# ChangwuLiu/InGVIO

Hardware: AMD Instinct MI355X
Metric: ekf_updates_per_sec (higher is better)
Workload: dtype f64; 1 GPU; BASELINE configs[1]: synthetic stereo MSCKF, 150 feats x 11 clones, state dim N=249 (update at N), 512 independent filters per GPU; step = propagate(k=10)+clone+MSCKF update+marginalise; filters_per_gpu=512, feats=150, clones=11, state_dim=249, imu_steps=10, parallelism=independent filters, 1 rank(s), no data-path collective

## Files before the change

include/ingvio_hip.h:

```cpp
#ifndef INGVIO_HIP_H
#define INGVIO_HIP_H

#include <stddef.h>

#ifdef __cplusplus
extern "C" {
#endif

#define INGVIO_OK 0
#define INGVIO_NO_ROWS 1
#define INGVIO_NEG_DIAG 2
#define INGVIO_REJECTED 3
#define INGVIO_E_ARG (-1)
#define INGVIO_E_CAPACITY (-2)
#define INGVIO_E_HIP (-3)
#define INGVIO_E_NOT_IN_STATE (-4)
#define INGVIO_E_UNSUPPORTED (-5)
#define INGVIO_E_NOT_PD (-6)

typedef struct ingvio_ctx ingvio_ctx;

typedef struct {
    int batch;
    int n_max;
// ... 302 lines not shown
    int track;
    int anchor;
    double pf[3];
} ingvio_lm_init_cand;
typedef struct {
    int n_cand; const ingvio_lm_init_cand* cand;
    int n_drop; const int* drop_cols;
} ingvio_lm_init_block;
int ingvio_landmark_init_nominal(ingvio_ctx* ctx, int b0, int nb, const ingvio_lm_init_block* blocks, const ingvio_msckf_opts* opts,
                                 double chi2_mult, int do_chi2, int cand_cap,
                                 int* added, int* new_idx, int* slot, double* chi2, double* dx, int* status);
int ingvio_debug_landmark_init_rows(ingvio_ctx* ctx, int b, const ingvio_lm_init_cand* cand, const ingvio_msckf_opts* opts,
                                    int n_drop, const int* drop_cols, double* H_old, double* H_new, double* res, int* m_out);
int ingvio_frame_run(ingvio_ctx* ctx, int restore_prior);
int ingvio_set_frame_parts(ingvio_ctx* ctx, int parts);
int ingvio_frame_fetch(ingvio_ctx* ctx, int b0, int nb, double* dx_out, int* accepted, int* rows_out);
int ingvio_frame_fetch_begin(ingvio_ctx* ctx, int b0, int nb);
int ingvio_frame_fetch_end(ingvio_ctx* ctx, double* dx_out, int* accepted, int* rows_out);

int ingvio_debug_msckf_info(ingvio_ctx* ctx, int b, double* A_out, int* ncol_out);

int ingvio_debug_info_solution(ingvio_ctx* ctx, int b, double* out, int count);

int ingvio_debug_tracks_read(ingvio_ctx* ctx, int b, unsigned long long* mask, double* uv, double* pf);

int ingvio_debug_staged_frame(ingvio_ctx* ctx, int b, int* n_clones, int* n_feat, int* clone_idx, double* clone_R, double* clone_p,
                              int* anchor, int* dof, unsigned long long* obs_mask, double* pf, double* uv);

int ingvio_debug_read(ingvio_ctx* ctx, long long* out, int n);

int ingvio_profile_enable(ingvio_ctx* ctx, int enable);
int ingvio_profile_select(ingvio_ctx* ctx, const char* kernel_name);
int ingvio_profile_reset(ingvio_ctx* ctx);
int ingvio_profile_get(ingvio_ctx* ctx, const char** names, double* ms, int* calls, int cap);

#ifdef __cplusplus
}
#endif
#endif
```

ingvio_amd/capi.py:

```python
import ctypes as C
import os

import numpy as np

_HERE = os.path.dirname(os.path.abspath(__file__))
LIB_PATH = os.environ.get("INGVIO_HIP_LIB") or os.path.join(_HERE, "lib", "libingvio_hip.so")

c_dp = C.POINTER(C.c_double)
c_ip = C.POINTER(C.c_int)
c_up = C.POINTER(C.c_ulonglong)

OK, NO_ROWS, NEG_DIAG, REJECTED = 0, 1, 2, 3
E_ARG, E_CAPACITY, E_HIP, E_NOT_IN_STATE, E_UNSUPPORTED, E_NOT_PD = -1, -2, -3, -4, -5, -6
R_SCALAR, R_DIAG, R_FULL = 0, 1, 2

EXPORTS = [
    "ingvio_ctx_create", "ingvio_ctx_destroy", "ingvio_sync", "ingvio_ctx_stream", "ingvio_f_max", "ingvio_c_max", "ingvio_last_error", "ingvio_ldp",
    "ingvio_build_id",
    "ingvio_cov_set", "ingvio_cov_get", "ingvio_get_n", "ingvio_cov_get_marginal", "ingvio_cov_snapshot",
    "ingvio_cov_restore", "ingvio_propagate", "ingvio_propagate_fused", "ingvio_augment_clone", "ingvio_marginalize",
    "ingvio_append_independent", "ingvio_ekf_update", "ingvio_chi2_gamma", "ingvio_msckf_update", "ingvio_msckf_update_tri", "ingvio_qr_compress",
    "ingvio_frame_stage", "ingvio_frame_stage_async", "ingvio_frame_set_imu_noise", "ingvio_frame_fetch_begin", "ingvio_frame_fetch_end", "ingvio_tracks_create", "ingvio_frame_stage_tracks", "ingvio_frame_run", "ingvio_set_frame_parts", "ingvio_frame_fetch", "ingvio_profile_enable", "ingvio_profile_select",
    "ingvio_profile_reset",
    "ingvio_profile_get", "ingvio_set_msckf_method", "ingvio_set_qr_method", "ingvio_landmark_stage", "ingvio_landmark_run",
    "ingvio_landmark_fetch", "ingvio_frame_run_phase", "ingvio_info_set", "ingvio_debug_read", "ingvio_triangulate",
    "ingvio_gnss_front_stage", "ingvio_gnss_front_fetch", "ingvio_gnss_update_batch", "ingvio_gnss_stage", "ingvio_gnss_run", "ingvio_gnss_fetch", "ingvio_mld", "ingvio_debug_msckf_info", "ingvio_debug_info_solution",
    "ingvio_info_reduce", "ingvio_info_commit", "ingvio_gnss_sat_eval",
    "ingvio_chi2_gamma_multi", "ingvio_ekf_update_batch", "ingvio_add_variable_delayed_invertible", "ingvio_add_variable_delayed", "ingvio_add_variable_delayed_batch", "ingvio_replace_var_linear",
    "ingvio_nominal_create", "ingvio_nominal_set", "ingvio_nominal_get", "ingvio_nominal_box_plus", "ingvio_frame_stage_tracks_nominal",
    "ingvio_nominal_set_gnss", "ingvio_nominal_get_gnss", "ingvio_gnss_front_stage_nominal", "ingvio_landmark_stage_nominal",
    "ingvio_landmark_init_nominal", "ingvio_debug_landmark_init_rows", "ingvio_nominal_tail",
    "ingvio_debug_tracks_read", "ingvio_debug_staged_frame",
]

NOM_NONE, NOM_SE23, NOM_SE3, NOM_VEC3, NOM_SCALAR, NOM_LANDMARK = -1, 0, 1, 2, 3, 4
NOM_VAL = 15

# ... 921 lines not shown
        fn = self.L.ingvio_frame_stage_async if use_async else self.L.ingvio_frame_stage

        def call(_keep=(keeps, chi2, sa, fa, o, sg)):
            self._chk(fn(self.h, b0, nb, sa, fa, C.byref(o), _d(sg), int(enable_gnss), C.c_double(sigma_cb), C.c_double(sigma_rw)))
        return call

    def frame_set_imu_noise(self, b0, noise):
        nz = f64(np.asarray(noise, dtype=np.float64).reshape(-1, 6))
        self._chk(self.L.ingvio_frame_set_imu_noise(self.h, int(b0), nz.shape[0], _d(nz)))

    def frame_run(self, restore_prior=False):
        self._chk(self.L.ingvio_frame_run(self.h, 1 if restore_prior else 0))

    def set_frame_parts(self, parts):
        self._chk(self.L.ingvio_set_frame_parts(self.h, int(parts)))

    def frame_fetch(self, b0=0, nb=None):
        nb = self.batch if nb is None else nb
        dx = np.zeros((nb, self.ldp)); acc = np.zeros((nb, self.f_max), dtype=np.int32); rows = np.zeros(nb, dtype=np.int32)
        self._chk(self.L.ingvio_frame_fetch(self.h, b0, nb, _d(dx), _i(acc), _i(rows)))
        return dx, acc, rows

    def frame_fetch_begin(self, b0=0, nb=None):
        nb = self.batch if nb is None else nb
        self._fetch_nb = nb
        self._chk(self.L.ingvio_frame_fetch_begin(self.h, b0, nb))

    def frame_fetch_end(self):
        nb = self._fetch_nb
        dx = np.empty((nb, self.ldp)); acc = np.empty((nb, self.f_max), dtype=np.int32); rows = np.empty(nb, dtype=np.int32)
# ... 85 lines not shown
```

ingvio_amd/csrc/capi.hip:

```cpp
#include "../../include/ingvio_hip.h"
#include "dev_common.h"
#include "launch_ekf.h"
#include "launch_msckf.h"
#include "launch_factored.h"
#include "launch_tri.h"
#include "launch_tracks.h"
#include "launch_lm.h"
#include "launch_delayed.h"
#include "launch_qr.h"
#include "launch_chol.h"
#include "launch_gnss.h"
#include "launch_lmbatch.h"
#include "launch_nominal.h"
#include "launch_tail.h"

#include <stdio.h>
#include <stdlib.h>
#include <string.h>
#include <unistd.h>
#include <string>
#include <atomic>
#include <cmath>
#include <condition_variable>
#include <functional>
// ... 123 lines not shown
    hipStream_t st2 = nullptr;
    hipEvent_t ev_fork = nullptr, ev_join = nullptr, ev_ref = nullptr;
    hipEvent_t ev_fetch = nullptr;
    int fetch_b0 = 0, fetch_nb = 0;
    hipStream_t st_copy = nullptr;
    hipEvent_t ev_copy = nullptr, ev_free[2] = { nullptr, nullptr };
    bool copy_pending = false, free_valid[2] = { false, false };
    int set_id = 0;
    struct PinSlab { char* p = nullptr; size_t cap = 0; hipEvent_t ev = nullptr; bool busy = false; };
    PinSlab pin[4];
    int pin_next = 0;
    struct PartStream { hipStream_t st = nullptr; hipEvent_t ev_gate = nullptr, ev_apply = nullptr, ev_done = nullptr; };
    PartStream part[4];
    int parts_alloc = 0;
    int parts_req = -1;
    bool split_pending = false;
    hipEvent_t tok_last = nullptr;
    hipEvent_t ev_split_fork = nullptr;
    hipStream_t run_st = nullptr;
    hipEvent_t tok_wait = nullptr, tok_rec = nullptr;
    struct Tracks { double *uv = nullptr, *pf = nullptr; unsigned long long* mask = nullptr; int t_max = 0; char* stage[2] = { nullptr, nullptr }; size_t stage_cap = 0; } trk;
    struct Nominal {
        int vmax = 0, ir = 0, dr = 0;
        int* ih = nullptr; double* dv = nullptr;
        int* ih_snap = nullptr; double* dv_snap = nullptr;
        double* dx = nullptr;
        std::vector<int> h_ih, h_ih_snap;
        bool has_snap = false;
        bool pending = false;
        bool frame = false;
// ... 547 lines not shown
    { ProfScope p(c, PF_EKF_CORE); launch_ekf_core(E, c->run_st); }
    L.gY = E.Y; L.gYstride = ws; L.gm = g.mf + b0;
    g.fused_last = true;
    g.results = true;
    return 0;
}

int run_msckf_factored(ingvio_ctx* c, int b0, int nb, const MsckfOpts& op, int stereo, int fmax_used,
                       const int* marg_idx = nullptr, int marg_size = 0, int phase = 0, bool gnss_fuse = false)
{
    FactoredLaunch L;
    memset(&L, 0, sizeof L);
    L.stereo = stereo; L.cv = view(c); L.fv = fview(c); L.op = op; L.b0 = b0; L.nb = nb;
    L.fmax_used = fmax_used > 0 ? fmax_used : 1;
    L.ncol_cap = 6 * c->d.c_max;
    for (int i = 0; i < nb; ++i) if (c->h_nclones[b0 + i] > L.c_used) L.c_used = c->h_nclones[b0 + i];
    L.gamma = c->d_gamma; L.accept = c->d_accept; L.used = c->d_used; L.rec = c->d_rec;
    L.Apart = c->d_Rpart + (size_t)b0 * c->G * c->rstride; L.chunk_used = c->d_chunk_used + (size_t)b0 * c->G;
    L.G = c->G; L.rstride = c->rstride; L.noise = c->d_noise + b0;
    L.Tflat = c->d_Tflat; L.tfstride = (size_t)c->ldp * 100; L.flat_nb = std::min(c->d.batch, APPLY_FLAT_NB);
    L.Asum = c->d_Asum ? c->d_Asum + (size_t)b0 * c->rstride : nullptr; L.used_sum = c->d_used_sum ? c->d_used_sum + b0 : nullptr;
#ifdef INGVIO_ALT_KERNELS
    static const bool few_off = [] { const char* e = getenv("INGVIO_FEW"); return e && !strcmp(e, "off"); }();
    if (few_off) { L.Tflat = nullptr; L.Asum = nullptr; }
#endif
    L.T = c->d_Y + (size_t)b0 * c->ystride; L.Pc = c->d_Yc + (size_t)b0 * c->ystride; L.ystride = c->ystride;
    L.dx = c->d_dx; L.m_out = c->d_m + b0; L.nc_out = c->d_nc + b0; L.status = c->d_status;
    L.big_sg = c->d_big_sg ? c->d_big_sg + (size_t)b0 * bigwin_sg_doubles(c->G) : nullptr;
    L.big_wk = c->d_big_wk ? c->d_big_wk + (size_t)b0 * bigwin_wk_doubles() : nullptr;
    const bool big = c->d.c_max > 16;
// ... 98 lines not shown
    if (desc->c_max > bigwin_cmax()) return INGVIO_E_CAPACITY;
    if (desc->m_max > 128) return INGVIO_E_CAPACITY;
    int ndev = 0;
    if (hipGetDeviceCount(&ndev) != hipSuccess || ndev <= desc->device) return INGVIO_E_HIP;
    ingvio_ctx* c = new ingvio_ctx();
    c->d = *desc;
    if (c->d.m_max < 1) c->d.m_max = 32;
    c->err.clear();
    if (hipSetDevice(desc->device) != hipSuccess) { delete c; return INGVIO_E_HIP; }
    c->own_stream = desc->stream == nullptr;
    if (c->own_stream) {
        if (hipStreamCreateWithFlags(&c->st, hipStreamNonBlocking) != hipSuccess) { delete c; return INGVIO_E_HIP; }
    } else c->st = (hipStream_t)desc->stream;
    c->run_st = c->st;
    if (const char* e = getenv("INGVIO_FRAME_PARTS")) c->parts_req = atoi(e);
    if (desc->c_max > 16) {
        int lo = 0, hi = 0;
        hipDeviceGetStreamPriorityRange(&lo, &hi);
        if (hipStreamCreateWithPriority(&c->st2, hipStreamNonBlocking, hi) != hipSuccess) c->st2 = nullptr;
        if (c->st2 && (hipEventCreateWithFlags(&c->ev_fork, hipEventDisableTiming) != hipSuccess ||
                       hipEventCreateWithFlags(&c->ev_ref, hipEventDisableTiming) != hipSuccess ||
                       hipEventCreateWithFlags(&c->ev_join, hipEventDisableTiming) != hipSuccess)) { hipStreamDestroy(c->st2); c->st2 = nullptr; }
    }
    const int B = desc->batch;
    c->ldp = (desc->n_max + 15) & ~15;
    const int cls0 = desc->c_max > 16 ? bigwin_cmax() : msckf_cmax_class(desc->c_max);
    const int cpad = cls0 > desc->c_max ? cls0 : desc->c_max;
    const int mcap = c->d.m_max > 6 * cpad ? c->d.m_max : 6 * cpad;
    c->mld = (mcap + 15) & ~15;
    c->nc_cap = c->ldp > mcap ? c->ldp : mcap;
// ... 2956 lines not shown
    if (c->alt_ready) {
        HIPCHK(c, hipEventRecord(c->ev_free[c->set_id], c->st));
        c->free_valid[c->set_id] = true;
    }
    return INGVIO_OK;
}

int ingvio_frame_run(ingvio_ctx* c, int restore_prior) { return frame_run_impl(c, restore_prior, 0); }
int ingvio_set_frame_parts(ingvio_ctx* c, int parts)
{
    if (!c || parts < -1 || parts > 4) return INGVIO_E_ARG;
    ENTER(c);
    c->parts_req = parts == 0 ? 1 : parts;
    return INGVIO_OK;
}
int ingvio_frame_run_phase(ingvio_ctx* c, int restore_prior, int phase)
{
    if (phase < 0 || phase > 2) return INGVIO_E_ARG;
    return frame_run_impl(c, restore_prior, phase);
}

int ingvio_info_set(ingvio_ctx* c, int b, const double* A, int ncol, int n_accepted)
{
    ENTER(c);
    if (check_range(c, b, 1) || !A || ncol < 6 || (size_t)ncol * (ncol + 1) > (size_t)c->rstride || n_accepted < 0) return INGVIO_E_ARG;
    std::vector<int> used(c->G, 0);
    used[0] = n_accepted;
    int rc = up(c, c->d_Rpart + (size_t)b * c->G * c->rstride, A, 8 * (size_t)ncol * (ncol + 1));
    rc |= up(c, c->d_chunk_used + (size_t)b * c->G, used.data(), sizeof(int) * (size_t)c->G);
    if (rc) return INGVIO_E_HIP;
// ... 191 lines not shown
    if (dbg_read_factored(a, 64) || dbg_read_cov(bq, 64) || dbg_read_bigwin(cq, 64) || dbg_read_solve(sq, 64)) return INGVIO_E_HIP;
    long long hq[64];
    if (dbg_read_chol(hq, 64)) return INGVIO_E_HIP;
    long long lq[64], mq[64];
    if (dbg_read_lmbatch(lq, 64) || dbg_read_lmchol(mq, 64)) return INGVIO_E_HIP;
    if (const char* e = getenv("INGVIO_DBG_TU")) {
        const long long* src = e[0] == 'b' ? cq : (e[0] == 'c' ? hq : (e[0] == 's' ? sq : (e[0] == 'l' ? lq : (e[0] == 'm' ? mq : a))));
        for (int i = 0; i < n; ++i) out[i] = src[i];
        return INGVIO_OK;
    }
    for (int i = 0; i < n; ++i)
        out[i] = i >= 56 ? hq[i - 56] : (i >= 48 ? cq[i] : ((i >= 24 && i < 32) ? sq[i - 24] : ((i < 16 || i >= 32) ? a[i] : bq[i])));
    return INGVIO_OK;
}

int ingvio_profile_select(ingvio_ctx* c, const char* kernel_name)
{
    ENTER(c);
    if (!c) return INGVIO_E_ARG;
    c->prof_only = -1;
    if (!kernel_name || !*kernel_name) return INGVIO_OK;
    for (int i = 0; i < PF_COUNT; ++i) if (!strcmp(kernel_name, kProfNames[i])) { c->prof_only = i; return INGVIO_OK; }
    return INGVIO_E_ARG;
}

int ingvio_profile_enable(ingvio_ctx* c, int enable)
{
    ENTER(c);
    if (!c) return INGVIO_E_ARG;
    c->prof = enable != 0;
// ... 35 lines not shown
```

ingvio_amd/csrc/dev_common.h:

```cpp
#pragma once
#include <hip/hip_runtime.h>
#include <stdint.h>

#define WAVE 64

struct CovView {
    double* Pbase;
    int* cur;
    int* n;
    int ldp;
    int B;
    size_t pstride;
};

__device__ __forceinline__ double* cov_ptr(const CovView& v, int b)
{
    return v.Pbase + ((size_t)v.cur[b] * v.B + b) * v.pstride;
}
__device__ __forceinline__ double* cov_alt_ptr(const CovView& v, int b)
{
    return v.Pbase + ((size_t)(1 - v.cur[b]) * v.B + b) * v.pstride;
}

struct FrameView {
// ... 19 lines not shown
    const double* chi2;
    int chi2_len;
};

__device__ __forceinline__ double wave_sum(double x)
{
#pragma unroll
    for (int off = 32; off > 0; off >>= 1) x += __shfl_xor(x, off, WAVE);
    return x;
}

__device__ __forceinline__ void lds_barrier()
{
    asm volatile("s_waitcnt lgkmcnt(0)\n\ts_barrier" ::: "memory");
}

template <int N>
__device__ __forceinline__ double row_ror_f64(double v)
{
    static_assert(N >= 1 && N <= 15, "row_ror");
#ifdef INGVIO_DPP32
    constexpr bool BC = false;
#else
    constexpr bool BC = true;
#endif
    const int lo = __builtin_amdgcn_update_dpp(0, __double2loint(v), 0x120 + N, 0xf, 0xf, BC);
    const int hi = __builtin_amdgcn_update_dpp(0, __double2hiint(v), 0x120 + N, 0xf, 0xf, BC);
    return __hiloint2double(hi, lo);
}

// ... 52 lines not shown
```

ingvio_amd/csrc/gram3_kernel.h:

```cpp
#pragma once

template <int CMAX>
struct Gram3Batch {
    using Cfg = Gram2Cfg<CMAX>;
    double Zm[2][Cfg::KR][Cfg::LDW];
    double sp[2][GRAM_NB][CMAX][Cfg::SPW];
};

template <int CMAX, bool STEREO>
__global__ __launch_bounds__(GRAM_NT, 2) void k_feat_gram3(
    FrameView fv, MsckfOpts op, int b0, const int* __restrict__ accept_in, int* __restrict__ used_out,
    double* __restrict__ Apart, int* __restrict__ chunk_used, int G, int rstride)
{
    using Cfg = Gram2Cfg<CMAX>;
    constexpr int NC = Cfg::NC, TJ = Cfg::TJ, LDW = Cfg::LDW, NTILE = Cfg::NTILE, TPW = Cfg::TPW, KR = Cfg::KR;
    constexpr int NUP = Cfg::NUP, TI = Cfg::TI, RPO = STEREO ? 4 : 2;
    extern __shared__ __attribute__((aligned(16))) char smem_raw[];
    static_assert(CMAX * CMAX <= 128, "the (slot, anchor) pair lanes sit on waves 2-3");
    Gram3Batch<CMAX>& sb = *reinterpret_cast<Gram3Batch<CMAX>*>(smem_raw);
    Gram2Out<CMAX>& so = *reinterpret_cast<Gram2Out<CMAX>*>(smem_raw);
    constexpr size_t UNI = sizeof(Gram3Batch<CMAX>) > sizeof(Gram2Out<CMAX>) ? sizeof(Gram3Batch<CMAX>) : sizeof(Gram2Out<CMAX>);
    int* sUse = reinterpret_cast<int*>(smem_raw + ((UNI + 15) / 16) * 16);
    int* sList = sUse + fv.fmax;
    __shared__ int sNu;
    __shared__ double sPose[16][12];
    const int bl = blockIdx.y, b = b0 + bl, g = blockIdx.x, tid = threadIdx.x, lane = tid & 63, wave = __builtin_amdgcn_readfirstlane(tid >> 6);
    const int F = fv.n_feat[b], C = fv.n_clones[b], ncol = 6 * C;
    for (int e = tid; e < 12 * C; e += GRAM_NT) {
        const int c = e / 12, q = e - 12 * c;
        sPose[c][q] = q < 9 ? fv.clone_R[((size_t)b * fv.cmax + c) * 9 + q] : fv.clone_p[((size_t)b * fv.cmax + c) * 3 + q - 9];
    }

    dbg_stamp(32);
    for (int j = tid; j < F; j += GRAM_NT) {
        int use = accept_in[(size_t)b * fv.fmax + j];
        if (use && op.max_accept > 0) {
            int rank = 0;
            for (int q = 0; q < j; ++q) rank += accept_in[(size_t)b * fv.fmax + q];
            if (rank >= op.max_accept) use = 0;
        }
        sUse[j] = use;
        if (g == 0) used_out[(size_t)b * fv.fmax + j] = use;
    }
    for (int e = tid; e < 2 * KR * LDW; e += GRAM_NT) (&sb.Zm[0][0][0])[e] = 0.0;
    __syncthreads();
    if (wave == 0) {
        int cnt = 0;
        for (int base = 0; base < F; base += WAVE) {
            const int j = base + lane;
            const bool u = j < F && sUse[j];
            const unsigned long long m = __ballot(u);
            if (u) sList[cnt + __popcll(m & ((1ULL << lane) - 1ULL))] = j;
            cnt += __popcll(m);
        }
        if (lane == 0) sNu = cnt;
    }
    __syncthreads();
    const int nu = sNu, per = (nu + G - 1) / G;
    const int q0 = g * per, q1 = min(nu, q0 + per);

    dbg_stamp(33);
    const int ptid = tid - 128;
    const int pc = ptid >= 0 ? ptid / CMAX : 0, pa = ptid >= 0 ? ptid - pc * CMAX : 0;
    const bool pairlane = ptid >= 0 && ptid < CMAX * CMAX;
    const int kq = lane >> 4, l15 = lane & 15;

    double in_uv[4], in_pf[3];
    unsigned long long in_mask = 0ULL;
    int in_anchor = 0;
    const int ft = tid;
    auto fetch = [&](int qb) {
        const int f = ft >> 4, c = ft & 15;
        in_mask = 0ULL; in_anchor = 0;
#pragma unroll
        for (int i = 0; i < 4; ++i) in_uv[i] = 0.0;
#pragma unroll
        for (int i = 0; i < 3; ++i) in_pf[i] = 0.0;
        if (ft < GRAM_NB * 16 && qb + f < q1) {
            const size_t oidx = (size_t)b * fv.fmax + sList[qb + f];
// ... 107 lines not shown
                }
              }
              if (sparse) {
                double* sp = sb.sp[buf][f][c < CMAX ? c : 0];
                double S1[9];
                mulXt(NX, px, py, pz, S1);
#pragma unroll
                for (int i = 0; i < 9; ++i) { sp[i] = cn * S1[i]; sp[9 + i] = cn * pl * NX[i]; }
                sp[18] = cn * (pz * h[1] - py * h[2]);
                sp[19] = cn * (px * h[2] - pz * h[0]);
                sp[20] = cn * (py * h[0] - px * h[1]);
#pragma unroll
                for (int i = 0; i < 9; ++i) sp[21 + i] = pl * N[i];
#pragma unroll
                for (int i = 0; i < 3; ++i) sp[30 + i] = pl * h[i];
                sp[33] = obs ? (double)a : -1.0;
              }
            }
        }
    };
    constexpr int N01 = (NUP + 2) / 3, N2 = (NUP - 2 * N01 + 1) / 2, N3 = NUP - 2 * N01 - N2;
    const int tcnt = wave < 2 ? N01 : (wave == 2 ? N2 : N3), tbeg = wave < 2 ? wave * N01 : (wave == 2 ? 2 * N01 : 2 * N01 + N2);
    int tiA[N01], tjA[N01];
#pragma unroll
    for (int u = 0; u < N01; ++u) {
        int t = u < tcnt ? tbeg + u : NUP, ti = 0;
        while (ti < TI - 1 && t >= TJ - ti) { t -= TJ - ti; ++ti; }
        tiA[u] = ti; tjA[u] = ti + t;
    }
    double4_f acc[N01];
#pragma unroll
    for (int u = 0; u < N01; ++u) acc[u] = double4_f{ 0.0, 0.0, 0.0, 0.0 };
    auto do_p3a = [&](int qb, int buf) {
        const int nbf = min(GRAM_NB, q1 - qb);
        const int nst = (3 * nbf + 3) >> 2;
#pragma unroll
        for (int st = 0; st < KR / 4; ++st) {
// ... 20 lines not shown
                for (int r = 0; r < 4; ++r) {
                    const int i = 16 * ti + kq + 4 * r;
                    if (i < NC && jc <= NC) so.A2[i][jc] = acc[u][r];
                }
            }
        }
    };
    if (wave < 2) {
        if (q0 < q1) { do_p2(q0, 0); fetch(q0 + GRAM_NB); }
        lds_barrier();
        int it = 0;
        for (int qb = q0; qb < q1; qb += GRAM_NB, ++it) {
            if (it == 3) dbg_stamp(36);
            if (qb + GRAM_NB < q1) { do_p2(qb + GRAM_NB, (it + 1) & 1); fetch(qb + 2 * GRAM_NB); }
            if (it == 3) dbg_stamp(37);
            do_p3a(qb, it & 1);
            if (it == 3) dbg_stamp(41);
            lds_barrier();
            if (it == 3) dbg_stamp(42);
        }
        store_acc();
    } else {
        double sS1[9], sNX[9], sS3[9], s4[3], s5[3];
#pragma unroll
        for (int i = 0; i < 9; ++i) { sS1[i] = 0.0; sNX[i] = 0.0; sS3[i] = 0.0; }
#pragma unroll
        for (int i = 0; i < 3; ++i) { s4[i] = 0.0; s5[i] = 0.0; }
        auto do_p3b = [&](int qb, int buf) {
            const int nbf = min(GRAM_NB, q1 - qb);
            if (pairlane) {
#pragma unroll
                for (int f = 0; f < GRAM_NB; ++f) {
                    if (f < nbf) {
                        const double* sp = sb.sp[buf][f][pc];
                        const double m = sp[33] == (double)pa ? 1.0 : 0.0;
#pragma unroll
                        for (int i = 0; i < 9; ++i) { sS1[i] = fma(m, sp[i], sS1[i]); sNX[i] = fma(m, sp[9 + i], sNX[i]); sS3[i] = fma(m, sp[21 + i], sS3[i]); }
#pragma unroll
                        for (int i = 0; i < 3; ++i) { s4[i] = fma(m, sp[18 + i], s4[i]); s5[i] = fma(m, sp[30 + i], s5[i]); }
                    }
                }
            }
        };
        lds_barrier();
        int it = 0;
        for (int qb = q0; qb < q1; qb += GRAM_NB, ++it) {
            do_p3a(qb, it & 1);
            do_p3b(qb, it & 1);
            lds_barrier();
        }
        store_acc();
        if (pairlane) {
            double* S = so.S[pc][pa];
#pragma unroll
            for (int i = 0; i < 9; ++i) { S[i] = sS1[i]; S[9 + i] = sNX[i]; S[18 + i] = sS3[i]; }
#pragma unroll
            for (int i = 0; i < 3; ++i) { S[27 + i] = s4[i]; S[30 + i] = s5[i]; }
        }
    }
    dbg_stamp(39);
    __syncthreads();
    double* out = Apart + ((size_t)bl * G + g) * rstride;
    if (pairlane && pc < C && pa < C) {
        const int c = pc, c2 = pa;
        double blk[36];
#pragma unroll
        for (int i = 0; i < 36; ++i) blk[i] = 0.0;
        double bb[6] = { 0.0, 0.0, 0.0, 0.0, 0.0, 0.0 };
        if (c == c2) {
            for (int a = 0; a < C; ++a) {
                const double* S = so.S[c][a];
                const double* Sa = so.S[a][c];
// ... 40 lines not shown
```

ingvio_amd/csrc/kernels_factored.hip:

```cpp
#include <algorithm>
#include <stdlib.h>
#include <string.h>
#include "launch_factored.h"

#include "gate_kernel.h"
#include "gate5_kernel.h"
#include "gate5m_kernel.h"

#define GATE_FPW 1
template <int CMAX, bool STEREO>
__global__ __launch_bounds__(GATE_FPW * WAVE) __attribute__((amdgpu_waves_per_eu(2, 4))) void k_feat_gate3(
    CovView cv, FrameView fv, MsckfOpts op, int b0, int nb, int fmax_used, double* __restrict__ gamma_out,
    int* __restrict__ accept_out, double* __restrict__ rec_out)
{
    gate3_body<CMAX, STEREO, GATE_FPW, false>(cv, fv, op, b0, nb, fmax_used, gamma_out, accept_out, rec_out);
}

#ifndef GATE4_WPE
#define GATE4_WPE 2
#endif
#ifndef GATE4_WPE_MAX
#define GATE4_WPE_MAX 6
#endif
template <int CMAX>
// ... 13 lines not shown
    gate5_body<CMAX>(cv, fv, op, b0, nb, fmax_used, gamma_out, accept_out);
}

template <int CMAX>
__global__ __launch_bounds__(WAVE) __attribute__((amdgpu_waves_per_eu(GATE5_WPE, GATE5_WPE))) void k_feat_gate5m(
    CovView cv, FrameView fv, MsckfOpts op, int b0, int nb, int fmax_used, double* __restrict__ gamma_out, int* __restrict__ accept_out)
{
    gate5m_body<CMAX>(cv, fv, op, b0, nb, fmax_used, gamma_out, accept_out);
}

#define GRAM_NB 8
#define GRAM_NT 256
#ifndef GRAM2_ZFORM
#define GRAM2_ZFORM 1
#endif
__device__ __forceinline__ double gram_rsqrt(double x)
{
    double y = __builtin_amdgcn_rsq(x);
    double e = fma(-x * y, y, 1.0);
    y = fma(y * e, fma(e, 0.375, 0.5), y);
    e = fma(-x * y, y, 1.0);
    return fma(y * e, 0.5, y);
}
template <int CMAX>
struct Gram2Cfg {
    static constexpr int NC = 6 * CMAX;
    static constexpr int TI = (NC + 15) / 16;
    static constexpr int TJ = (NC + 1 + 15) / 16;
    static constexpr int LDW = 16 * TJ;
    static constexpr int NTILE = TI * TJ;
// ... 7 lines not shown
    using Cfg = Gram2Cfg<CMAX>;
    double Bm[Cfg::KR][Cfg::LDW];
    double Ym[Cfg::KR][Cfg::LDW];
    double sp[CMAX * CMAX <= 128 ? 2 : 1][GRAM_NB][CMAX][Cfg::SPW];
};
template <int CMAX>
struct Gram2Out {
    using Cfg = Gram2Cfg<CMAX>;
    double A2[Cfg::NC][Cfg::NC + 2];
    double S[CMAX][CMAX][34];
};

template <int CMAX, bool STEREO>
__global__ __launch_bounds__(GRAM_NT, 2) void k_feat_gram2(
    FrameView fv, MsckfOpts op, int b0, const int* __restrict__ accept_in, int* __restrict__ used_out,
    double* __restrict__ Apart, int* __restrict__ chunk_used, int G, int rstride)
{
    using Cfg = Gram2Cfg<CMAX>;
    constexpr int NC = Cfg::NC, TJ = Cfg::TJ, LDW = Cfg::LDW, NTILE = Cfg::NTILE, TPW = Cfg::TPW, KR = Cfg::KR;
    constexpr int NUP = Cfg::NUP, TI = Cfg::TI, RPO = STEREO ? 4 : 2;
    extern __shared__ __attribute__((aligned(16))) char smem_raw[];
    Gram2Batch<CMAX>& sb = *reinterpret_cast<Gram2Batch<CMAX>*>(smem_raw);
    Gram2Out<CMAX>& so = *reinterpret_cast<Gram2Out<CMAX>*>(smem_raw);
    constexpr size_t UNI = sizeof(Gram2Batch<CMAX>) > sizeof(Gram2Out<CMAX>) ? sizeof(Gram2Batch<CMAX>) : sizeof(Gram2Out<CMAX>);
    int* sUse = reinterpret_cast<int*>(smem_raw + ((UNI + 15) / 16) * 16);
    int* sList = sUse + fv.fmax;
    __shared__ int sNu;
    __shared__ double sPose[16][12];
    const int bl = blockIdx.y, b = b0 + bl, g = blockIdx.x, tid = threadIdx.x, lane = tid & 63, wave = __builtin_amdgcn_readfirstlane(tid >> 6);
    const int F = fv.n_feat[b], C = fv.n_clones[b], ncol = 6 * C;
    for (int e = tid; e < 12 * C; e += GRAM_NT) {
        const int c = e / 12, q = e - 12 * c;
        sPose[c][q] = q < 9 ? fv.clone_R[((size_t)b * fv.cmax + c) * 9 + q] : fv.clone_p[((size_t)b * fv.cmax + c) * 3 + q - 9];
    }

    dbg_stamp(32);
    for (int j = tid; j < F; j += GRAM_NT) {
        int use = accept_in[(size_t)b * fv.fmax + j];
        if (use && op.max_accept > 0) {
            int rank = 0;
            for (int q = 0; q < j; ++q) rank += accept_in[(size_t)b * fv.fmax + q];
            if (rank >= op.max_accept) use = 0;
        }
        sUse[j] = use;
        if (g == 0) used_out[(size_t)b * fv.fmax + j] = use;
    }
    for (int e = tid; e < KR * LDW; e += GRAM_NT) { (&sb.Bm[0][0])[e] = 0.0; (&sb.Ym[0][0])[e] = 0.0; }
    __syncthreads();
    if (wave == 0) {
        int cnt = 0;
        for (int base = 0; base < F; base += WAVE) {
            const int j = base + lane;
            const bool u = j < F && sUse[j];
            const unsigned long long m = __ballot(u);
            if (u) sList[cnt + __popcll(m & ((1ULL << lane) - 1ULL))] = j;
            cnt += __popcll(m);
        }
        if (lane == 0) sNu = cnt;
    }
    __syncthreads();
    const int nu = sNu, per = (nu + G - 1) / G;
    const int q0 = g * per, q1 = min(nu, q0 + per);

// ... 1073 lines not shown
        LAUNCH_GATE(L, (k_feat_gate3<CMAX, STEREO>), dim3(nb8 * ((L.fmax_used + GATE_FPW - 1) / GATE_FPW)), dim3(GATE_FPW * WAVE), 0, st,
                           L.cv, L.fv, L.op, L.b0, L.nb, L.fmax_used, L.gamma, L.accept, L.rec);
    } else {
#ifdef INGVIO_ALT_KERNELS
        if constexpr (CMAX * CMAX <= 128) {
            static const bool gram3 = [] { const char* e = getenv("INGVIO_GRAM"); return e && e[0] == '3'; }();
            if (gram3) {
                constexpr size_t uni3 = sizeof(Gram3Batch<CMAX>) > sizeof(Gram2Out<CMAX>) ? sizeof(Gram3Batch<CMAX>) : sizeof(Gram2Out<CMAX>);
                const size_t sm3 = ((uni3 + 15) / 16) * 16 + 2 * sizeof(int) * (size_t)L.fv.fmax;
                static size_t attr_sm3 = 0;
                if (sm3 > attr_sm3) {
                    hipFuncSetAttribute((const void*)k_feat_gram3<CMAX, STEREO>, hipFuncAttributeMaxDynamicSharedMemorySize, (int)sm3);
                    attr_sm3 = sm3;
                }
                hipLaunchKernelGGL((k_feat_gram3<CMAX, STEREO>), dim3(L.G, L.nb), dim3(GRAM_NT), sm3, st,
                                   L.fv, L.op, L.b0, L.accept, L.used, L.Apart, L.chunk_used, L.G, L.rstride);
                return;
            }
        }
#endif
        constexpr size_t uni = sizeof(Gram2Batch<CMAX>) > sizeof(Gram2Out<CMAX>) ? sizeof(Gram2Batch<CMAX>) : sizeof(Gram2Out<CMAX>);
        const size_t sm = ((uni + 15) / 16) * 16 + 2 * sizeof(int) * (size_t)L.fv.fmax;
        static size_t attr_sm = 0;
        if (sm > attr_sm) {
            hipFuncSetAttribute((const void*)k_feat_gram2<CMAX, STEREO>, hipFuncAttributeMaxDynamicSharedMemorySize, (int)sm);
            attr_sm = sm;
        }
        hipLaunchKernelGGL((k_feat_gram2<CMAX, STEREO>), dim3(L.G, L.nb), dim3(GRAM_NT), sm, st,
                           L.fv, L.op, L.b0, L.accept, L.used, L.Apart, L.chunk_used, L.G, L.rstride);
    }
}

__global__ __launch_bounds__(256) void k_chunk_sum(const double* __restrict__ Apart, const int* __restrict__ chunk_used, int G, int rstride,
                                                   double* __restrict__ out, int* __restrict__ used_out)
{
    const int bl = blockIdx.y, e = blockIdx.x * 256 + threadIdx.x;
    const int* cu = chunk_used + (size_t)bl * G;
    const double* A = Apart + (size_t)bl * G * rstride;
    unsigned long long mask = 0;
    int total = 0;
    for (int g = 0; g < G; ++g) { mask |= (cu[g] != 0 ? 1ull : 0ull) << g; total += cu[g]; }
    if (e < rstride) {
        double s = 0.0;
#pragma unroll 8
// ... 86 lines not shown
    }
    const int cm = cm_sel;
    const int cls = cm <= 6 ? 6 : (cm <= 11 ? 11 : (cm <= 12 ? 12 : (cm <= 16 ? 16 : -1)));
    if (cls < 0) return -1;
#define DISPATCH(CM)                                                         \
    if (cls == CM) { if (L.stereo) launch_ft<CM, true>(L, st); else launch_ft<CM, false>(L, st); return 0; }
    DISPATCH(6)
    DISPATCH(11)
    DISPATCH(12)
    DISPATCH(16)
#undef DISPATCH
    return -1;
}

int dbg_read_factored(long long* out, int n) { return dbg_read_local(out, n); }
```

ingvio_amd/csrc/launch_factored.h:

```cpp
#pragma once
#include "dev_common.h"

#ifndef INGVIO_APPLY_FLAT_NB
#define INGVIO_APPLY_FLAT_NB 64
#endif
constexpr int APPLY_FLAT_NB = INGVIO_APPLY_FLAT_NB;

struct FactoredLaunch {
    int stage;
    int stereo;
    CovView cv;
    FrameView fv;
    MsckfOpts op;
    int b0, nb, fmax_used;
    double* gamma;
    int* accept;
    int* used;
    double* rec;
    double* Apart;
    double* Asum;
    int* used_sum;
    double* Tflat;
    size_t tfstride;
    int flat_nb;
// ... 15 lines not shown
    int* did_flip;
    double* big_sg;
    double* big_wk;
    int ncol_cap;
    int c_used;
    const int* gcolmap;
    const int* gnc;
    int gcstride;
    double* gW;
    size_t gWstride;
    const double* gY;
    size_t gYstride;
    const int* gm;
    hipEvent_t prof_a, prof_b;
    int* prof_used;
};
#include <hip/hip_ext.h>
#define LAUNCH_GATE(L, kernel, grid, block, shmem, st, ...)                                                             \
    do {                                                                                                                \
        if ((L).prof_a) { hipExtLaunchKernelGGL(kernel, grid, block, shmem, st, (L).prof_a, (L).prof_b, 0, __VA_ARGS__); if ((L).prof_used) *(L).prof_used = 1; } \
        else hipLaunchKernelGGL(kernel, grid, block, shmem, st, __VA_ARGS__);                                           \
    } while (0)

int launch_factored(const FactoredLaunch& L, hipStream_t st);
int launch_info_solve(const FactoredLaunch& L, hipStream_t st);
int dbg_read_solve(long long* out, int n);
int factored_rec_size(int cmax);
int dbg_read_factored(long long* out, int n);

int launch_bigwin(const FactoredLaunch& L, hipStream_t st);
void launch_apply64(const FactoredLaunch& L, hipStream_t st, int mp, double* T, size_t tstride, int ldt);
size_t bigwin_sg_doubles(int G);
size_t bigwin_wk_doubles();
int bigwin_rec_size();
int bigwin_cmax();
int dbg_read_bigwin(long long* out, int n);
```

Measured before the change: 1.071 million updates/s.

## Rebalance gram3 wave roles and add SIMD-aware logical wave remapping

Adds an optional remapping of physical waves to logical roles based on hardware SIMD id and LDS base, exposed via an API call and environment variable, plus a placement debug probe. In gram3 the tile accumulation moves entirely onto waves 2-3 by default (GRAM3_TILES23), so waves 0-1 skip do_p3a and store_acc. The anchor-sum lanes are restructured from (clone, anchor) pairs to (clone, chunk) lanes that accumulate across all anchors with a wave-uniform anchor index. The aim is better balance between SIMDs and cheaper per-feature reductions, at the cost of more registers (3*CMAX accumulators) and a modified sp[33] encoding.

```diff
diff --git a/include/ingvio_hip.h b/include/ingvio_hip.h
--- a/include/ingvio_hip.h
+++ b/include/ingvio_hip.h
@@ -340,6 +340,7 @@
                                     int n_drop, const int* drop_cols, double* H_old, double* H_new, double* res, int* m_out);
 int ingvio_frame_run(ingvio_ctx* ctx, int restore_prior);
 int ingvio_set_frame_parts(ingvio_ctx* ctx, int parts);
+int ingvio_set_gram_roles(ingvio_ctx* ctx, int mode);
 int ingvio_frame_fetch(ingvio_ctx* ctx, int b0, int nb, double* dx_out, int* accepted, int* rows_out);
 int ingvio_frame_fetch_begin(ingvio_ctx* ctx, int b0, int nb);
 int ingvio_frame_fetch_end(ingvio_ctx* ctx, double* dx_out, int* accepted, int* rows_out);
@@ -354,6 +355,7 @@
                               int* anchor, int* dof, unsigned long long* obs_mask, double* pf, double* uv);
 
 int ingvio_debug_read(ingvio_ctx* ctx, long long* out, int n);
+int ingvio_debug_gram_placement(ingvio_ctx* ctx, long long* out, int n);
 
 int ingvio_profile_enable(ingvio_ctx* ctx, int enable);
 int ingvio_profile_select(ingvio_ctx* ctx, const char* kernel_name);
diff --git a/ingvio_amd/capi.py b/ingvio_amd/capi.py
--- a/ingvio_amd/capi.py
+++ b/ingvio_amd/capi.py
@@ -20,7 +20,7 @@
     "ingvio_cov_set", "ingvio_cov_get", "ingvio_get_n", "ingvio_cov_get_marginal", "ingvio_cov_snapshot",
     "ingvio_cov_restore", "ingvio_propagate", "ingvio_propagate_fused", "ingvio_augment_clone", "ingvio_marginalize",
     "ingvio_append_independent", "ingvio_ekf_update", "ingvio_chi2_gamma", "ingvio_msckf_update", "ingvio_msckf_update_tri", "ingvio_qr_compress",
-    "ingvio_frame_stage", "ingvio_frame_stage_async", "ingvio_frame_set_imu_noise", "ingvio_frame_fetch_begin", "ingvio_frame_fetch_end", "ingvio_tracks_create", "ingvio_frame_stage_tracks", "ingvio_frame_run", "ingvio_set_frame_parts", "ingvio_frame_fetch", "ingvio_profile_enable", "ingvio_profile_select",
+    "ingvio_frame_stage", "ingvio_frame_stage_async", "ingvio_frame_set_imu_noise", "ingvio_frame_fetch_begin", "ingvio_frame_fetch_end", "ingvio_tracks_create", "ingvio_frame_stage_tracks", "ingvio_frame_run", "ingvio_set_frame_parts", "ingvio_set_gram_roles", "ingvio_debug_gram_placement", "ingvio_frame_fetch", "ingvio_profile_enable", "ingvio_profile_select",
     "ingvio_profile_reset",
     "ingvio_profile_get", "ingvio_set_msckf_method", "ingvio_set_qr_method", "ingvio_landmark_stage", "ingvio_landmark_run",
     "ingvio_landmark_fetch", "ingvio_frame_run_phase", "ingvio_info_set", "ingvio_debug_read", "ingvio_triangulate",
@@ -972,6 +972,14 @@
 
     def set_frame_parts(self, parts):
         self._chk(self.L.ingvio_set_frame_parts(self.h, int(parts)))
+
+    def set_gram_roles(self, mode):
+        self._chk(self.L.ingvio_set_gram_roles(self.h, int(mode)))
+
+    def debug_gram_placement(self, n_wg):
+        out = (C.c_longlong * (8 * n_wg))()
+        self._chk(self.L.ingvio_debug_gram_placement(self.h, out, 8 * n_wg))
+        return np.array(out, dtype=np.int64).reshape(n_wg, 4, 2)
 
     def frame_fetch(self, b0=0, nb=None):
         nb = self.batch if nb is None else nb
diff --git a/ingvio_amd/csrc/capi.hip b/ingvio_amd/csrc/capi.hip
--- a/ingvio_amd/csrc/capi.hip
+++ b/ingvio_amd/csrc/capi.hip
@@ -161,6 +161,7 @@
     PartStream part[4];
     int parts_alloc = 0;
     int parts_req = -1;
+    int gram_roles_req = -1;
     bool split_pending = false;
     hipEvent_t tok_last = nullptr;
     hipEvent_t ev_split_fork = nullptr;
@@ -738,6 +739,7 @@
     L.stereo = stereo; L.cv = view(c); L.fv = fview(c); L.op = op; L.b0 = b0; L.nb = nb;
     L.fmax_used = fmax_used > 0 ? fmax_used : 1;
     L.ncol_cap = 6 * c->d.c_max;
+    L.gram_roles = c->gram_roles_req < 0 ? GRAM_ROLES_AUTO : c->gram_roles_req;
     for (int i = 0; i < nb; ++i) if (c->h_nclones[b0 + i] > L.c_used) L.c_used = c->h_nclones[b0 + i];
     L.gamma = c->d_gamma; L.accept = c->d_accept; L.used = c->d_used; L.rec = c->d_rec;
     L.Apart = c->d_Rpart + (size_t)b0 * c->G * c->rstride; L.chunk_used = c->d_chunk_used + (size_t)b0 * c->G;
@@ -866,6 +868,7 @@
     } else c->st = (hipStream_t)desc->stream;
     c->run_st = c->st;
     if (const char* e = getenv("INGVIO_FRAME_PARTS")) c->parts_req = atoi(e);
+    if (const char* e = getenv("INGVIO_GRAM_ROLES")) { const int m = atoi(e); c->gram_roles_req = m < 0 ? -1 : (m > 0 ? 1 : 0); }
     if (desc->c_max > 16) {
         int lo = 0, hi = 0;
         hipDeviceGetStreamPriorityRange(&lo, &hi);
@@ -3852,6 +3855,13 @@
     c->parts_req = parts == 0 ? 1 : parts;
     return INGVIO_OK;
 }
+int ingvio_set_gram_roles(ingvio_ctx* c, int mode)
+{
+    if (!c || mode < -1 || mode > 1) return INGVIO_E_ARG;
+    ENTER(c);
+    c->gram_roles_req = mode;
+    return INGVIO_OK;
+}
 int ingvio_frame_run_phase(ingvio_ctx* c, int restore_prior, int phase)
 {
     if (phase < 0 || phase > 2) return INGVIO_E_ARG;
@@ -4073,6 +4083,15 @@
     return INGVIO_OK;
 }
 
+int ingvio_debug_gram_placement(ingvio_ctx* c, long long* out, int n)
+{
+    ENTER(c);
+    if (!c || !out || n < 1) return INGVIO_E_ARG;
+    HIPCHK(c, hipStreamSynchronize(c->st));
+    const int r = dbg_read_gram_place(out, n);
+    return r < 0 ? INGVIO_E_UNSUPPORTED : (r ? INGVIO_E_HIP : INGVIO_OK);
+}
+
 int ingvio_profile_select(ingvio_ctx* c, const char* kernel_name)
 {
     ENTER(c);
diff --git a/ingvio_amd/csrc/dev_common.h b/ingvio_amd/csrc/dev_common.h
--- a/ingvio_amd/csrc/dev_common.h
+++ b/ingvio_amd/csrc/dev_common.h
@@ -57,6 +57,13 @@
 {
     asm volatile("s_waitcnt lgkmcnt(0)\n\ts_barrier" ::: "memory");
 }
+
+#define INGVIO_GETREG(id, off, size) __builtin_amdgcn_s_getreg((((size) - 1) << 11) | ((off) << 6) | (id))
+__device__ __forceinline__ unsigned hw_reg_hw_id() { return INGVIO_GETREG(4, 0, 32); }
+__device__ __forceinline__ unsigned hw_reg_lds_alloc() { return INGVIO_GETREG(6, 0, 32); }
+__device__ __forceinline__ unsigned hw_reg_xcc_id() { return INGVIO_GETREG(20, 0, 4); }
+__device__ __forceinline__ int hw_simd_id() { return (int)INGVIO_GETREG(4, 4, 2); }
+__device__ __forceinline__ int hw_lds_base() { return (int)INGVIO_GETREG(6, 0, 8); }
 
 template <int N>
 __device__ __forceinline__ double row_ror_f64(double v)
diff --git a/ingvio_amd/csrc/gram3_kernel.h b/ingvio_amd/csrc/gram3_kernel.h
--- a/ingvio_amd/csrc/gram3_kernel.h
+++ b/ingvio_amd/csrc/gram3_kernel.h
@@ -10,7 +10,7 @@
 template <int CMAX, bool STEREO>
 __global__ __launch_bounds__(GRAM_NT, 2) void k_feat_gram3(
     FrameView fv, MsckfOpts op, int b0, const int* __restrict__ accept_in, int* __restrict__ used_out,
-    double* __restrict__ Apart, int* __restrict__ chunk_used, int G, int rstride)
+    double* __restrict__ Apart, int* __restrict__ chunk_used, int G, int rstride, int roles)
 {
     using Cfg = Gram2Cfg<CMAX>;
     constexpr int NC = Cfg::NC, TJ = Cfg::TJ, LDW = Cfg::LDW, NTILE = Cfg::NTILE, TPW = Cfg::TPW, KR = Cfg::KR;
@@ -24,15 +24,17 @@
     int* sList = sUse + fv.fmax;
     __shared__ int sNu;
     __shared__ double sPose[16][12];
-    const int bl = blockIdx.y, b = b0 + bl, g = blockIdx.x, tid = threadIdx.x, lane = tid & 63, wave = __builtin_amdgcn_readfirstlane(tid >> 6);
+    __shared__ int sRole[5];
+    const int bl = blockIdx.y, b = b0 + bl, g = blockIdx.x, tid0 = threadIdx.x, lane = tid0 & 63, wave0 = __builtin_amdgcn_readfirstlane(tid0 >> 6);
     const int F = fv.n_feat[b], C = fv.n_clones[b], ncol = 6 * C;
-    for (int e = tid; e < 12 * C; e += GRAM_NT) {
+    gram_roles_publish(sRole, wave0, lane);
+    for (int e = tid0; e < 12 * C; e += GRAM_NT) {
         const int c = e / 12, q = e - 12 * c;
         sPose[c][q] = q < 9 ? fv.clone_R[((size_t)b * fv.cmax + c) * 9 + q] : fv.clone_p[((size_t)b * fv.cmax + c) * 3 + q - 9];
     }
 
     dbg_stamp(32);
-    for (int j = tid; j < F; j += GRAM_NT) {
+    for (int j = tid0; j < F; j += GRAM_NT) {
         int use = accept_in[(size_t)b * fv.fmax + j];
         if (use && op.max_accept > 0) {
             int rank = 0;
@@ -42,8 +44,9 @@
         sUse[j] = use;
         if (g == 0) used_out[(size_t)b * fv.fmax + j] = use;
     }
-    for (int e = tid; e < 2 * KR * LDW; e += GRAM_NT) (&sb.Zm[0][0][0])[e] = 0.0;
+    for (int e = tid0; e < 2 * KR * LDW; e += GRAM_NT) (&sb.Zm[0][0][0])[e] = 0.0;
     __syncthreads();
+    const int wave = gram_logical_wave(sRole, wave0, roles), tid = 64 * wave + lane;
     if (wave == 0) {
         int cnt = 0;
         for (int base = 0; base < F; base += WAVE) {
@@ -63,6 +66,9 @@
     const int ptid = tid - 128;
     const int pc = ptid >= 0 ? ptid / CMAX : 0, pa = ptid >= 0 ? ptid - pc * CMAX : 0;
     const bool pairlane = ptid >= 0 && ptid < CMAX * CMAX;
+    static_assert(11 * CMAX <= 128, "the (slot, chunk) lanes sit on waves 2-3");
+    const int uc = ptid >= 0 ? ptid / 11 : 0, uj = ptid >= 0 ? ptid - 11 * uc : 0;
+    const bool ulane = ptid >= 0 && ptid < 11 * CMAX;
     const int kq = lane >> 4, l15 = lane & 15;
 
     double in_uv[4], in_pf[3];
@@ -200,13 +206,18 @@
                 for (int i = 0; i < 9; ++i) sp[21 + i] = pl * N[i];
 #pragma unroll
                 for (int i = 0; i < 3; ++i) sp[30 + i] = pl * h[i];
-                sp[33] = obs ? (double)a : -1.0;
+                sp[33] = (obs || c == 0) ? (double)a : -1.0;
               }
             }
         }
     };
-    constexpr int N01 = (NUP + 2) / 3, N2 = (NUP - 2 * N01 + 1) / 2, N3 = NUP - 2 * N01 - N2;
-    const int tcnt = wave < 2 ? N01 : (wave == 2 ? N2 : N3), tbeg = wave < 2 ? wave * N01 : (wave == 2 ? 2 * N01 : 2 * N01 + N2);
+#ifndef GRAM3_TILES23
+#define GRAM3_TILES23 1
+#endif
+    constexpr bool T23 = GRAM3_TILES23 != 0;
+    constexpr int N01r = T23 ? 0 : (NUP + 2) / 3, N2 = (NUP - 2 * N01r + 1) / 2, N3 = NUP - 2 * N01r - N2;
+    constexpr int N01 = N01r > N2 ? N01r : N2;
+    const int tcnt = wave < 2 ? N01r : (wave == 2 ? N2 : N3), tbeg = wave < 2 ? wave * N01r : (wave == 2 ? 2 * N01r : 2 * N01r + N2);
     int tiA[N01], tjA[N01];
 #pragma unroll
     for (int u = 0; u < N01; ++u) {
@@ -257,30 +268,32 @@
             if (it == 3) dbg_stamp(36);
             if (qb + GRAM_NB < q1) { do_p2(qb + GRAM_NB, (it + 1) & 1); fetch(qb + 2 * GRAM_NB); }
             if (it == 3) dbg_stamp(37);
-            do_p3a(qb, it & 1);
+            if constexpr (!T23) do_p3a(qb, it & 1);
             if (it == 3) dbg_stamp(41);
             lds_barrier();
             if (it == 3) dbg_stamp(42);
         }
-        store_acc();
+        if constexpr (!T23) store_acc();
     } else {
-        double sS1[9], sNX[9], sS3[9], s4[3], s5[3];
-#pragma unroll
-        for (int i = 0; i < 9; ++i) { sS1[i] = 0.0; sNX[i] = 0.0; sS3[i] = 0.0; }
-#pragma unroll
-        for (int i = 0; i < 3; ++i) { s4[i] = 0.0; s5[i] = 0.0; }
+        double sacc[3 * CMAX];
+#pragma unroll
+        for (int i = 0; i < 3 * CMAX; ++i) sacc[i] = 0.0;
         auto do_p3b = [&](int qb, int buf) {
             const int nbf = min(GRAM_NB, q1 - qb);
-            if (pairlane) {
+            if (ulane) {
 #pragma unroll
                 for (int f = 0; f < GRAM_NB; ++f) {
                     if (f < nbf) {
-                        const double* sp = sb.sp[buf][f][pc];
-                        const double m = sp[33] == (double)pa ? 1.0 : 0.0;
-#pragma unroll
-                        for (int i = 0; i < 9; ++i) { sS1[i] = fma(m, sp[i], sS1[i]); sNX[i] = fma(m, sp[9 + i], sNX[i]); sS3[i] = fma(m, sp[21 + i], sS3[i]); }
-#pragma unroll
-                        for (int i = 0; i < 3; ++i) { s4[i] = fma(m, sp[18 + i], s4[i]); s5[i] = fma(m, sp[30 + i], s5[i]); }
+                        const double* sp = sb.sp[buf][f][uc];
+                        const int af = __builtin_amdgcn_readfirstlane((int)sb.sp[buf][f][0][33]);
+                        const double x0 = sp[3 * uj], x1 = sp[3 * uj + 1], x2 = sp[3 * uj + 2];
+#pragma unroll
+                        for (int a2 = 0; a2 < CMAX; ++a2) {
+                            const double m = af == a2 ? 1.0 : 0.0;
+                            sacc[3 * a2] = fma(m, x0, sacc[3 * a2]);
+                            sacc[3 * a2 + 1] = fma(m, x1, sacc[3 * a2 + 1]);
+                            sacc[3 * a2 + 2] = fma(m, x2, sacc[3 * a2 + 2]);
+                        }
                     }
                 }
             }
@@ -293,12 +306,14 @@
             lds_barrier();
         }
         store_acc();
-        if (pairlane) {
-            double* S = so.S[pc][pa];
-#pragma unroll
-            for (int i = 0; i < 9; ++i) { S[i] = sS1[i]; S[9 + i] = sNX[i]; S[18 + i] = sS3[i]; }
-#pragma unroll
-            for (int i = 0; i < 3; ++i) { S[27 + i] = s4[i]; S[30 + i] = s5[i]; }
+        if (ulane) {
+#pragma unroll
+            for (int a2 = 0; a2 < CMAX; ++a2)
+#pragma unroll
+                for (int i = 0; i < 3; ++i) {
+                    const int v = 3 * uj + i;
+                    so.S[uc][a2][v < 18 ? v : (v < 21 ? v + 9 : (v < 30 ? v - 3 : v))] = sacc[3 * a2 + i];
+                }
         }
     }
     dbg_stamp(39);
diff --git a/ingvio_amd/csrc/kernels_factored.hip b/ingvio_amd/csrc/kernels_factored.hip
--- a/ingvio_amd/csrc/kernels_factored.hip
+++ b/ingvio_amd/csrc/kernels_factored.hip
@@ -51,6 +51,43 @@
 #ifndef GRAM2_ZFORM
 #define GRAM2_ZFORM 1
 #endif
+#define GRAM_PLACE_WG 1024
+#ifdef INGVIO_DBG_STAMPS
+static __device__ long long g_gram_place[GRAM_PLACE_WG * 8];
+#endif
+__device__ __forceinline__ void gram_place_probe(int wave0, int lwave)
+{
+#ifdef INGVIO_DBG_STAMPS
+    const unsigned wg = blockIdx.y * gridDim.x + blockIdx.x;
+    if ((threadIdx.x & 63) == 0 && wg < GRAM_PLACE_WG) {
+        g_gram_place[wg * 8 + 2 * wave0] = (long long)(((unsigned long long)hw_reg_lds_alloc() << 32) | hw_reg_hw_id());
+        g_gram_place[wg * 8 + 2 * wave0 + 1] = (long long)(hw_reg_xcc_id() | ((unsigned)lwave << 8) | (1u << 16));
+    }
+#else
+    (void)wave0; (void)lwave;
+#endif
+}
+__device__ __forceinline__ void gram_roles_publish(int* sRole, int wave0, int lane)
+{
+    if (lane == 0) {
+        sRole[wave0] = hw_simd_id();
+        if (wave0 == 0) sRole[4] = hw_lds_base() != 0 ? 1 : 0;
+    }
+}
+__device__ __forceinline__ int gram_logical_wave(const int* sRole, int wave0, int roles)
+{
+    if (!roles) return wave0;
+    const int par = __builtin_amdgcn_readfirstlane(sRole[4]);
+    int seen = 0, mine = 0;
+#pragma unroll
+    for (int w = 0; w < 4; ++w) {
+        const int sd = __builtin_amdgcn_readfirstlane(sRole[w]);
+        const int lw = ((((sd & 1) ^ par) == 0) ? 0 : 2) + ((sd >> 1) & 1);
+        seen |= 1 << lw;
+        if (w == wave0) mine = lw;
+    }
+    return seen == 15 ? __builtin_amdgcn_readfirstlane(mine) : wave0;
+}
 __device__ __forceinline__ double gram_rsqrt(double x)
 {
     double y = __builtin_amdgcn_rsq(x);
@@ -88,7 +125,7 @@
 template <int CMAX, bool STEREO>
 __global__ __launch_bounds__(GRAM_NT, 2) void k_feat_gram2(
     FrameView fv, MsckfOpts op, int b0, const int* __restrict__ accept_in, int* __restrict__ used_out,
-    double* __restrict__ Apart, int* __restrict__ chunk_used, int G, int rstride)
+    double* __restrict__ Apart, int* __restrict__ chunk_used, int G, int rstride, int roles)
 {
     using Cfg = Gram2Cfg<CMAX>;
     constexpr int NC = Cfg::NC, TJ = Cfg::TJ, LDW = Cfg::LDW, NTILE = Cfg::NTILE, TPW = Cfg::TPW, KR = Cfg::KR;
@@ -101,15 +138,17 @@
     int* sList = sUse + fv.fmax;
     __shared__ int sNu;
     __shared__ double sPose[16][12];
-    const int bl = blockIdx.y, b = b0 + bl, g = blockIdx.x, tid = threadIdx.x, lane = tid & 63, wave = __builtin_amdgcn_readfirstlane(tid >> 6);
+    __shared__ int sRole[5];
+    const int bl = blockIdx.y, b = b0 + bl, g = blockIdx.x, tid0 = threadIdx.x, lane = tid0 & 63, wave0 = __builtin_amdgcn_readfirstlane(tid0 >> 6);
     const int F = fv.n_feat[b], C = fv.n_clones[b], ncol = 6 * C;
-    for (int e = tid; e < 12 * C; e += GRAM_NT) {
+    gram_roles_publish(sRole, wave0, lane);
+    for (int e = tid0; e < 12 * C; e += GRAM_NT) {
         const int c = e / 12, q = e - 12 * c;
         sPose[c][q] = q < 9 ? fv.clone_R[((size_t)b * fv.cmax + c) * 9 + q] : fv.clone_p[((size_t)b * fv.cmax + c) * 3 + q - 9];
     }
 
     dbg_stamp(32);
-    for (int j = tid; j < F; j += GRAM_NT) {
+    for (int j = tid0; j < F; j += GRAM_NT) {
         int use = accept_in[(size_t)b * fv.fmax + j];
         if (use && op.max_accept > 0) {
             int rank = 0;
@@ -119,8 +158,10 @@
         sUse[j] = use;
         if (g == 0) used_out[(size_t)b * fv.fmax + j] = use;
     }
-    for (int e = tid; e < KR * LDW; e += GRAM_NT) { (&sb.Bm[0][0])[e] = 0.0; (&sb.Ym[0][0])[e] = 0.0; }
+    for (int e = tid0; e < KR * LDW; e += GRAM_NT) { (&sb.Bm[0][0])[e] = 0.0; (&sb.Ym[0][0])[e] = 0.0; }
     __syncthreads();
+    const int wave = gram_logical_wave(sRole, wave0, roles), tid = 64 * wave + lane;
+    gram_place_probe(wave0, wave);
     if (wave == 0) {
         int cnt = 0;
         for (int base = 0; base < F; base += WAVE) {
@@ -1224,7 +1265,7 @@
                     attr_sm3 = sm3;
                 }
                 hipLaunchKernelGGL((k_feat_gram3<CMAX, STEREO>), dim3(L.G, L.nb), dim3(GRAM_NT), sm3, st,
-                                   L.fv, L.op, L.b0, L.accept, L.used, L.Apart, L.chunk_used, L.G, L.rstride);
+                                   L.fv, L.op, L.b0, L.accept, L.used, L.Apart, L.chunk_used, L.G, L.rstride, L.gram_roles);
                 return;
             }
         }
@@ -1237,7 +1278,7 @@
             attr_sm = sm;
         }
         hipLaunchKernelGGL((k_feat_gram2<CMAX, STEREO>), dim3(L.G, L.nb), dim3(GRAM_NT), sm, st,
-                           L.fv, L.op, L.b0, L.accept, L.used, L.Apart, L.chunk_used, L.G, L.rstride);
+                           L.fv, L.op, L.b0, L.accept, L.used, L.Apart, L.chunk_used, L.G, L.rstride, L.gram_roles);
     }
 }
 
@@ -1354,3 +1395,13 @@
 }
 
 int dbg_read_factored(long long* out, int n) { return dbg_read_local(out, n); }
+int dbg_read_gram_place(long long* out, int n)
+{
+#ifdef INGVIO_DBG_STAMPS
+    if (n > GRAM_PLACE_WG * 8) return 1;
+    return (int)hipMemcpyFromSymbol(out, HIP_SYMBOL(g_gram_place), sizeof(long long) * n);
+#else
+    (void)out; (void)n;
+    return -1;
+#endif
+}
diff --git a/ingvio_amd/csrc/launch_factored.h b/ingvio_amd/csrc/launch_factored.h
--- a/ingvio_amd/csrc/launch_factored.h
+++ b/ingvio_amd/csrc/launch_factored.h
@@ -53,6 +53,7 @@
     const int* gm;
     hipEvent_t prof_a, prof_b;
     int* prof_used;
+    int gram_roles;
 };
 #include <hip/hip_ext.h>
 #define LAUNCH_GATE(L, kernel, grid, block, shmem, st, ...)                                                             \
@@ -61,11 +62,13 @@
         else hipLaunchKernelGGL(kernel, grid, block, shmem, st, __VA_ARGS__);                                           \
     } while (0)
 
+#define GRAM_ROLES_AUTO 0
 int launch_factored(const FactoredLaunch& L, hipStream_t st);
 int launch_info_solve(const FactoredLaunch& L, hipStream_t st);
 int dbg_read_solve(long long* out, int n);
 int factored_rec_size(int cmax);
 int dbg_read_factored(long long* out, int n);
+int dbg_read_gram_place(long long* out, int n);
 
 int launch_bigwin(const FactoredLaunch& L, hipStream_t st);
 void launch_apply64(const FactoredLaunch& L, hipStream_t st, int mp, double* T, size_t tstride, int ldt);
```

Measured after the change: 1.068 million updates/s. About the same (-0.2%).
